# CFD-Xing/gpu-benchmarking

Measured on AMD Instinct MI355X. Metric: GDOF/s for 3D hex sum-factorisation, fp64, nq=2..10 sweep, higher is better.
Workload: dtype f64

## Files before the change

gpu-benchmarking_amd/csrc/bwdtrans_hex.hip:

```cpp
#include "sf_dispatch.h"
#include "wave_launch.h"
#include "wave_table.h"

#include <cstdlib>

namespace sf
{

template <int NQ> struct HexSmall
{
    static constexpr int EC  = HexCfg<NQ>::EC == 1 ? 1
                               : ((HexCfg<NQ>::EC / 4 + 1) / 2 * 2 < 2 ? 2 : (HexCfg<NQ>::EC / 4 + 1) / 2 * 2);
    static constexpr int OUT = HexCfg<NQ>::OUT;
};

__global__ __launch_bounds__(256) void hex_nq2_stream_kernel(const double *__restrict__ b0,
                                                             const double *__restrict__ b1,
                                                             const double *__restrict__ b2,
                                                             const double *__restrict__ in,
                                                             double *__restrict__ out, uint64_t nelmt)
{
    constexpr int U   = 1;
    const uint64_t nv = nelmt * 4;
    const double c0 = b0[0], c1 = b0[1];
    double2_t *out2 = reinterpret_cast<double2_t *>(out);
    const uint64_t base = logical_block<64>() * (256ull * U) + threadIdx.x;
#pragma unroll
    for (int u = 0; u < U; ++u)
    {
        const uint64_t v = base + (uint64_t)u * 256;
        if (v < nv)
        {
            const int p    = (int)(v & 3);
            const double x = in[v >> 2];
            const double bj = b1[p & 1], bk = b2[p >> 1];
            const double2_t r = {((x * c0) * bj) * bk, ((x * c1) * bj) * bk};
            __builtin_nontemporal_store(r, out2 + v);
        }
    }
}

static int launch_hex_nq2(const HexArgs &a, hipStream_t s)
{
    if (a.nelmt == 0)
        return SF_OK;
    const uint64_t blocks = (a.nelmt * 4 + 255) / 256;
    if (blocks > 0x7fffffffull)
        return SF_EINVAL;
    hex_nq2_stream_kernel<<<(unsigned)blocks, 256, 0, s>>>(a.b0, a.b1, a.b2, a.in, a.out, a.nelmt);
    hipError_t e = hipGetLastError();
    return e == hipSuccess ? SF_OK : (int)e;
}

template <int NQ> static int go(const HexArgs &a, hipStream_t s)
{
    if constexpr (NQ == 2)
        return launch_hex_nq2(a, s);
    using C = HexCfg<NQ>;
    constexpr uint64_t per_block = (uint64_t)C::EC * C::WPB * (C::KM > 0 ? C::KM : 1);
    if (a.nelmt < 2 * per_block * (uint64_t)device_info().num_cu)
        return launch_hex_wave<NQ, HexSmall<NQ>::EC, 1, C::BM, C::MW, 1, HexSmall<NQ>::OUT>(a, s);
    constexpr uint64_t piece = hex_piece(NQ);
    if (piece > 0 && a.nelmt > 2 * piece)
    {
        static_assert(piece == 0 || piece % (8 * 64 * per_block) == 0, "pieces hold whole XCD windows");
        constexpr uint64_t NMT = (uint64_t)(NQ - 1) * (NQ - 1) * (NQ - 1), NQT = (uint64_t)NQ * NQ * NQ;
        for (uint64_t lo = 0; lo < a.nelmt; lo += piece)
        {
            HexArgs part = a;
            part.in      = a.in + lo * NMT;
            part.out     = a.out + lo * NQT;
            part.nelmt   = a.nelmt - lo < piece ? a.nelmt - lo : piece;
            const int rc = launch_hex_wave<NQ, C::EC, C::WPB, C::BM, C::MW, C::KM, C::OUT, C::MF>(part, s);
            if (rc != SF_OK)
                return rc;
        }
        return SF_OK;
    }
    return launch_hex_wave<NQ, C::EC, C::WPB, C::BM, C::MW, C::KM, C::OUT, C::MF>(a, s);
}

int launch_hex_wave_nq(unsigned nq, const HexArgs &a, hipStream_t s)
{
    switch (nq)
    {
    case 2: return go<2>(a, s);
    case 3: return go<3>(a, s);
    case 4: return go<4>(a, s);
    case 5: return go<5>(a, s);
    case 6: return go<6>(a, s);
    case 7: return go<7>(a, s);
    case 8: return go<8>(a, s);
    case 9: return go<9>(a, s);
    case 10: return go<10>(a, s);
    case 11: return go<11>(a, s);
    default: return SF_ENOTBUILT;
    }
}

template <int NQ> static int go_mfma(const HexArgs &a, hipStream_t s)
{
    if constexpr (NQ <= 10)
        return launch_hex_mfma<NQ, 2, 2, 2, 1>(a, s);
    else
    {
        constexpr int WPB = NQ == 11 ? 4 : 1;
        constexpr int MW  = (NQ == 14 || NQ == 15) ? 2 : 1;
        return launch_hex_mfma<NQ, 1, WPB, MW, 1, 64>(a, s);
    }
}

int launch_hex_mfma_nq(unsigned nq, const HexArgs &a, hipStream_t s)
{
    switch (nq)
    {
    case 4: return go_mfma<4>(a, s);
    case 5: return go_mfma<5>(a, s);
    case 6: return go_mfma<6>(a, s);
    case 7: return go_mfma<7>(a, s);
    case 8: return go_mfma<8>(a, s);
    case 9: return go_mfma<9>(a, s);
    case 10: return go_mfma<10>(a, s);
    case 11: return go_mfma<11>(a, s);
    case 12: return go_mfma<12>(a, s);
    case 13: return go_mfma<13>(a, s);
    case 14: return go_mfma<14>(a, s);
    case 15: return go_mfma<15>(a, s);
    case 16: return go_mfma<16>(a, s);
    default: return SF_ENOTBUILT;
    }
}

template <int NQ> static int go_mfma4(const HexArgs &a, hipStream_t s)
{
    const char *env = getenv("SF_HEX_MFMA4_CFG");
    const int cfg   = env ? atoi(env) : (NQ == 16 ? 3 : 1);
    if (cfg == 3)
        return launch_hex_mfma4<NQ, 1, 2, 1, 64, true>(a, s);
    return launch_hex_mfma4<NQ, 1, (NQ == 12 ? 1 : 2), 1, 64>(a, s);
}

int launch_hex_mfma4_nq(unsigned nq, const HexArgs &a, hipStream_t s)
{
    switch (nq)
    {
    case 12: return go_mfma4<12>(a, s);
    case 13: return go_mfma4<13>(a, s);
    case 14: return go_mfma4<14>(a, s);
    case 15: return go_mfma4<15>(a, s);
    case 16: return go_mfma4<16>(a, s);
    default: return SF_ENOTBUILT;
    }
}

int hex_auto_kernel(unsigned nq)
{
    return (nq == 12 || nq == 14 || nq == 16) ? SF_VARIANT_MFMA4 : SF_VARIANT_MFMA;
}

typedef float float4_t __attribute__((ext_vector_type(4)));
__global__ __launch_bounds__(256) void hex_nq2_stream_f32_kernel(const float *__restrict__ b0, const float *__restrict__ b1,
                                                                 const float *__restrict__ b2, const float *__restrict__ in,
                                                                 float *__restrict__ out, uint64_t nelmt)
{
    const uint64_t nv = nelmt * 2;
    const uint64_t v  = logical_block<64>() * 256ull + threadIdx.x;
    if (v < nv)
    {
        const float x  = in[v >> 1];
        const float bk = b2[v & 1];
        const float x0 = x * b0[0], x1 = x * b0[1];
        const float4_t r = {(x0 * b1[0]) * bk, (x1 * b1[0]) * bk, (x0 * b1[1]) * bk, (x1 * b1[1]) * bk};
        __builtin_nontemporal_store(r, reinterpret_cast<float4_t *>(out) + v);
    }
}

template <int NQ> static int go_f32(const HexArgsT<float> &a, hipStream_t s)
{
    if constexpr (NQ == 2)
    {
        if (a.nelmt == 0)
            return SF_OK;
        const uint64_t blocks = (a.nelmt * 2 + 255) / 256;
        if (blocks > 0x7fffffffull)
            return SF_EINVAL;
        hex_nq2_stream_f32_kernel<<<(unsigned)blocks, 256, 0, s>>>(a.b0, a.b1, a.b2, a.in, a.out, a.nelmt);
        hipError_t e = hipGetLastError();
        return e == hipSuccess ? SF_OK : (int)e;
    }
    if constexpr (NQ >= 12)
    {
        constexpr int best = NQ == 12 ? 0 : (NQ <= 14 ? 2 : 1);
        static const int cfg = getenv("SF_F32_HEX_CFG") ? atoi(getenv("SF_F32_HEX_CFG")) : best;
        switch (cfg)
        {
        case 1: return launch_hex_mfma<NQ, 1, 1, 1, 1, 64, float>(a, s);
        case 2: return launch_hex_mfma<NQ, 1, 1, 2, 1, 64, float>(a, s);
        case 3: return launch_hex_mfma<NQ, 1, 2, 2, 1, 64, float>(a, s);
        case 4: return launch_hex_mfma<NQ, 2, 1, 1, 1, 64, float>(a, s);
        default: break;
        }
    }
    using C = HexCfgF32<NQ>;
    return launch_hex_wave<NQ, C::EC, C::WPB, C::BM, C::MW, C::KM, C::OUT, C::MF, float>(a, s);
}

int launch_hex_wave_f32_nq(unsigned nq, const HexArgsT<float> &a, hipStream_t s)
{
    switch (nq)
    {
    case 2: return go_f32<2>(a, s);
    case 3: return go_f32<3>(a, s);
    case 4: return go_f32<4>(a, s);
    case 5: return go_f32<5>(a, s);
    case 6: return go_f32<6>(a, s);
    case 7: return go_f32<7>(a, s);
    case 8: return go_f32<8>(a, s);
    case 9: return go_f32<9>(a, s);
    case 10: return go_f32<10>(a, s);
    case 11: return go_f32<11>(a, s);
    case 12: return go_f32<12>(a, s);
    case 13: return go_f32<13>(a, s);
    case 14: return go_f32<14>(a, s);
    case 15: return go_f32<15>(a, s);
    case 16: return go_f32<16>(a, s);
    default: return SF_ENOTBUILT;
    }
}

}
```

gpu-benchmarking_amd/csrc/bwdtrans_wave.h:

```cpp
#pragma once

#include "sf_common.h"

namespace sf
{

enum OutMode
{
    OUT_ST8  = 0,
    OUT_ST16 = 1,
    OUT_LDS  = 2
};

enum BasisMode
{
    BASIS_LDS = 0,
    BASIS_SMEM = 1,
    BASIS_SMEM_COLS = 2,
    BASIS_SMEM_COLS16 = 3
};

template <typename T> struct VecOf
{
    static constexpr int W = 16 / (int)sizeof(T);
    typedef T type __attribute__((ext_vector_type(W)));
};

__device__ __forceinline__ double fma_t(double a, double b, double c)
{
    return __builtin_fma(a, b, c);
}
__device__ __forceinline__ float fma_t(float a, float b, float c)
{
    return __builtin_fmaf(a, b, c);
}

__device__ __forceinline__ double swap_adjacent(double v)
{
    int lo = __double2loint(v), hi = __double2hiint(v);
    lo     = __builtin_amdgcn_mov_dpp(lo, 0xB1, 0xF, 0xF, true);
    hi     = __builtin_amdgcn_mov_dpp(hi, 0xB1, 0xF, 0xF, true);
    return __hiloint2double(hi, lo);
}

template <int NQ, int EC, int DIM, typename T = double> struct WaveGeom
{
    using Scalar = T;
    using Vec    = typename VecOf<T>::type;
    static constexpr int VW  = VecOf<T>::W;
    static constexpr int NM  = NQ - 1;
    static constexpr int NMP = NM | 1;
    static constexpr int NMT = (DIM == 3) ? NM * NM * NM : NM * NM;
    static constexpr int NQT = (DIM == 3) ? NQ * NQ * NQ : NQ * NQ;
    static constexpr int IN_STRIDE = (NM % 2 == 0) ? NM + 1 : NM;
    static constexpr int IN_DBL    = EC * NMT;
    static constexpr bool VEC2     = (IN_DBL % VW) == 0;
    static constexpr int P0 = (DIM == 3) ? EC * NM * NM : EC * NM;
    static constexpr int P1 = (DIM == 3) ? EC * NQ * NM : EC * NQ;
    static constexpr int P2 = EC * NQ * NQ;
    static constexpr int PASS0 = cdiv(P0, kWave);
    static constexpr int PASS1 = cdiv(P1, kWave);
    static constexpr int PASS2 = cdiv(P2, kWave);
    static constexpr int SLAB_IN = P0 * IN_STRIDE;
    static constexpr int SLAB_W1 = P1 * NMP;
    static constexpr int SLAB_W2 = (DIM == 3) ? P2 * NMP : 0;
    static constexpr int SLAB0   = CMax<CMax<SLAB_IN, SLAB_W1>::value, SLAB_W2>::value;
    static constexpr int OUT_DBL = EC * NQT;
    static constexpr int SLAB_NOOUT = (SLAB0 + VW - 1) / VW * VW;
    static constexpr int SLAB_OUT   = (CMax<SLAB0, OUT_DBL>::value + VW - 1) / VW * VW;
    static constexpr int NBAS = (NM * NQ + VW - 1) / VW * VW;
    static constexpr int NLD  = VEC2 ? cdiv(IN_DBL / VW, kWave) : cdiv(IN_DBL, kWave);
    static constexpr bool ALIGN_OK = VEC2 && cdiv(IN_DBL / VW + 7, kWave) == NLD;
};

__device__ __forceinline__ int align_shift(const void *p)
{
    return __builtin_amdgcn_readfirstlane((int)(((uintptr_t)p >> 4) & 7));
}

template <class G, int OUTM> constexpr int slab_doubles()
{
    return OUTM == OUT_LDS ? G::SLAB_OUT : G::SLAB_NOOUT;
}

template <int NQ, int EC, int DIM, int WPB, int BMODE, int OUTM, typename T = double>
constexpr size_t wave_lds_bytes()
{
    using G = WaveGeom<NQ, EC, DIM, T>;
    return sizeof(T) *
           (size_t)((BMODE == BASIS_LDS ? DIM * G::NBAS : 0) + WPB * slab_doubles<G, OUTM>());
}

struct ChunkIter
{
    uint64_t first, step, count;
};

template <int KMAP, int WPB, int XG = 0>
__device__ __forceinline__ ChunkIter chunk_iter(uint64_t nchunk, int wib)
{
    const uint64_t gw = logical_block<XG>() * WPB + wib;
    ChunkIter it;
    if constexpr (KMAP == 0)
    {
        const uint64_t nwave = (uint64_t)gridDim.x * WPB;
        it.first = gw;
        it.step  = nwave;
        it.count = gw < nchunk ? (nchunk - gw + nwave - 1) / nwave : 0;
    }
    else if constexpr (KMAP > 0)
    {
        it.first = gw * KMAP;
        it.step  = 1;
        it.count = it.first < nchunk ? (nchunk - it.first < KMAP ? nchunk - it.first : KMAP) : 0;
    }
    else
    {
        constexpr int K     = -KMAP;
        const uint64_t base = logical_block<XG>() * WPB * K;
        it.first            = base + wib;
        it.step             = WPB;
        const uint64_t end  = base + (uint64_t)WPB * K < nchunk ? base + (uint64_t)WPB * K : nchunk;
        it.count            = it.first < end ? (end - it.first + WPB - 1) / WPB : 0;
    }
    return it;
}

template <typename T> __device__ __forceinline__ int line_offset(const void *p)
{
    return __builtin_amdgcn_readfirstlane((int)(((uintptr_t)p / sizeof(T)) & (128 / sizeof(T) - 1)));
}
__device__ __forceinline__ int line_offset_f64(const void *p)
{
    return line_offset<double>(p);
}

template <int NMAX, typename T> constexpr int word_grid_regs()
{
    return cdiv(NMAX + (int)(128 / sizeof(T)) - 1, (int)(16 / sizeof(T)) * kWave);
}

template <int NMAX, int NREG, typename T>
__device__ __forceinline__ void chunk_load_any(typename VecOf<T>::type (&st)[NREG], const T *__restrict__ src,
                                               int lane, int nvalid)
{
    using V          = typename VecOf<T>::type;
    constexpr int VW = VecOf<T>::W;
    constexpr int NLDA = word_grid_regs<NMAX, T>();
    static_assert(NLDA <= NREG, "staging registers");
    const int a   = line_offset<T>(src);
    const V *grid = reinterpret_cast<const V *>(src - a);
#pragma unroll
    for (int k = 0; k < NLDA; ++k)
    {
        const int gv = k * kWave + lane;
        const int d0 = VW * gv - a;
        V x          = {};
        if (d0 >= 0 && d0 + VW - 1 < nvalid)
            x = __builtin_nontemporal_load(grid + gv);
        else
        {
#pragma unroll
            for (int h = 0; h < VW; ++h)
                if (d0 + h >= 0 && d0 + h < nvalid)
                    x[h] = src[d0 + h];
        }
        st[k] = x;
    }
}

template <int NMAX, int NREG>
__device__ __forceinline__ void chunk_load_any_f64(double2_t (&st)[NREG], const double *__restrict__ src,
                                                   int lane, int nvalid)
{
    chunk_load_any<NMAX, NREG, double>(st, src, lane, nvalid);
}

template <typename V, int N> __device__ __forceinline__ void touch_staged(V (&st)[N])
{
#pragma unroll
    for (int k = 0; k < N; ++k)
        asm volatile("" : "+v"(st[k]));
}

template <class G, bool FULL, bool NTL = true, bool AL = false>
__device__ __forceinline__ void chunk_load(typename G::Vec (&st)[G::NLD],
                                           const typename G::Scalar *__restrict__ src, int lane,
                                           int nvalid )
{
    using T = typename G::Scalar;
    using V = typename G::Vec;
    constexpr int VW = G::VW;
    if constexpr (G::VEC2)
    {
        const V *srcv = reinterpret_cast<const V *>(src);
        const int sh  = AL ? align_shift(src) : 0;
#pragma unroll
        for (int k = 0; k < G::NLD; ++k)
        {
            const int v = k * kWave + lane - sh;
            if constexpr (FULL)
            {
                if (AL ? (v >= 0 && v < G::IN_DBL / VW)
                       : ((k + 1) * kWave <= G::IN_DBL / VW || v < G::IN_DBL / VW))
                    st[k] = NTL ? __builtin_nontemporal_load(srcv + v) : srcv[v];
            }
            else
            {
                V x = {};
                if (AL && v < 0)
                    ;
                else if (VW * v + VW - 1 < nvalid)
                    x = NTL ? __builtin_nontemporal_load(srcv + v) : srcv[v];
                else
                {
#pragma unroll
                    for (int j = 0; j < VW - 1; ++j)
                        if (VW * v + j < nvalid)
                            x[j] = src[VW * v + j];
                }
                st[k] = x;
            }
        }
    }
    else
    {
        chunk_load_any<G::IN_DBL, G::NLD, T>(st, src, lane, FULL ? G::IN_DBL : nvalid);
    }
}

template <class G, bool AL = false>
__device__ __forceinline__ void chunk_stage(const typename G::Vec (&st)[G::NLD],
                                            typename G::Scalar *slab, int lane, int sh = 0)
{
    using V = typename G::Vec;
    constexpr int VW = G::VW;
    if constexpr (G::VEC2)
    {
#pragma unroll
        for (int k = 0; k < G::NLD; ++k)
        {
            const int v = k * kWave + lane - (AL ? sh : 0);
            if (AL ? (v >= 0 && v < G::IN_DBL / VW)
                   : ((k + 1) * kWave <= G::IN_DBL / VW || v < G::IN_DBL / VW))
            {
                if constexpr (G::IN_STRIDE == G::NM)
                {
                    *reinterpret_cast<V *>(slab + VW * v) = st[k];
                }
                else
                {
#pragma unroll
                    for (int j = 0; j < VW; ++j)
                    {
                        const int f          = VW * v + j;
                        slab[f + f / G::NM] = st[k][j];
                    }
                }
            }
        }
    }
    else
    {
#pragma unroll
        for (int k = 0; k < word_grid_regs<G::IN_DBL, typename G::Scalar>(); ++k)
#pragma unroll
            for (int h = 0; h < VW; ++h)
            {
                const int f = VW * (k * kWave + lane) - sh + h;
                if (f >= 0 && f < G::IN_DBL)
                {
                    if constexpr (G::IN_STRIDE == G::NM)
                        slab[f] = st[k][h];
                    else
                        slab[f + f / G::NM] = st[k][h];
                }
            }
    }
}

typedef float float2_t __attribute__((ext_vector_type(2)));
template <int NB, int N0, int NOUT, int NPASS>
__device__ __forceinline__ void fma_row(bool first, const double (&um)[NPASS], const double (&b)[NB],
                                        double (&acc)[NPASS][NOUT])
{
#pragma unroll
    for (int n = 0; n < NB; ++n)
#pragma unroll
        for (int s = 0; s < NPASS; ++s)
            acc[s][N0 + n] = first ? um[s] * b[n] : fma_t(um[s], b[n], acc[s][N0 + n]);
}
template <int NB, int N0, int NOUT, int NPASS>
__device__ __forceinline__ void fma_row(bool first, const float (&um)[NPASS], const float (&b)[NB],
                                        float (&acc)[NPASS][NOUT])
{
    constexpr int NPAIR = (NOUT >= 9 && NOUT <= 24) ? NB / 2 : 0;
#pragma unroll
    for (int n = 0; n < 2 * NPAIR; n += 2)
#pragma unroll
        for (int s = 0; s < NPASS; ++s)
        {
            const float2_t uu = {um[s], um[s]}, bb = {b[n], b[n + 1]};
            const float2_t a  = {acc[s][N0 + n], acc[s][N0 + n + 1]};
            const float2_t r  = first ? uu * bb : __builtin_elementwise_fma(uu, bb, a);
            acc[s][N0 + n]     = r.x;
            acc[s][N0 + n + 1] = r.y;
        }
#pragma unroll
    for (int n = 2 * NPAIR; n < NB; ++n)
#pragma unroll
        for (int s = 0; s < NPASS; ++s)
            acc[s][N0 + n] = first ? um[s] * b[n] : fma_t(um[s], b[n], acc[s][N0 + n]);
}

template <int NIN, int NOUT, int NPASS, int N0, int kColBlock, typename T>
__device__ __forceinline__ void contract_cols(const T (&u)[NPASS][NIN], T (&acc)[NPASS][NOUT],
                                              const T *__restrict__ bas, int &zero)
{
    constexpr int NB = (NOUT - N0) < kColBlock ? (NOUT - N0) : kColBlock;
    T b[2][NB];
#pragma unroll
    for (int n = 0; n < NB; ++n)
        b[0][n] = bas[zero + N0 + n];
#pragma unroll
    for (int m = 0; m < NIN; ++m)
    {
#pragma unroll
        for (int n = 0; n < NB; ++n)
            asm volatile("" : "+s"(zero) : "s"(b[m % 2][n]));
        if (m + 1 < NIN)
        {
#pragma unroll
            for (int n = 0; n < NB; ++n)
                b[(m + 1) % 2][n] = bas[zero + (m + 1) * NOUT + N0 + n];
            __builtin_amdgcn_sched_barrier(0);
        }
        {
            T um[NPASS];
#pragma unroll
            for (int s = 0; s < NPASS; ++s)
                um[s] = u[s][m];
            fma_row<NB, N0>(m == 0, um, b[m % 2], acc);
        }
#pragma unroll
        for (int n = 0; n < NB; ++n)
#pragma unroll
            for (int s = 0; s < NPASS; ++s)
                asm volatile("" : "+s"(zero) : "v"(acc[s][N0 + n]));
    }
    if constexpr (N0 + NB < NOUT)
        contract_cols<NIN, NOUT, NPASS, N0 + NB, kColBlock, T>(u, acc, bas, zero);
}

template <int NIN, int NOUT, int NPASS, int BMODE, typename T>
__device__ __forceinline__ void contract(const T (&u)[NPASS][NIN], T (&acc)[NPASS][NOUT],
                                         const T *__restrict__ bas)
{
    if constexpr (BMODE == BASIS_SMEM_COLS || BMODE == BASIS_SMEM_COLS16)
    {
        int z = 0;
        asm volatile("s_mov_b32 %0, 0" : "=s"(z));
        contract_cols<NIN, NOUT, NPASS, 0, (BMODE == BASIS_SMEM_COLS ? 8 : 16), T>(u, acc, bas, z);
        return;
    }
    int zero = 0;
    asm volatile("s_mov_b32 %0, 0" : "=s"(zero));
    constexpr int RING = 2;
    T b[RING][NOUT];
#pragma unroll
    for (int n = 0; n < NOUT; ++n)
        b[0][n] = bas[zero + n];
#pragma unroll
    for (int m = 0; m < NIN; ++m)
    {
        if constexpr (BMODE == BASIS_SMEM)
        {
#pragma unroll
            for (int n = 0; n < NOUT; ++n)
                asm volatile("" : "+s"(zero) : "s"(b[m % RING][n]));
        }
        if (m + 1 < NIN)
        {
#pragma unroll
            for (int n = 0; n < NOUT; ++n)
                b[(m + 1) % RING][n] = bas[zero + (m + 1) * NOUT + n];
            __builtin_amdgcn_sched_barrier(0);
        }
        {
            T um[NPASS];
#pragma unroll
            for (int s = 0; s < NPASS; ++s)
                um[s] = u[s][m];
            fma_row<NOUT, 0>(m == 0, um, b[m % RING], acc);
        }
#pragma unroll
        for (int n = 0; n < NOUT; ++n)
#pragma unroll
            for (int s = 0; s < NPASS; ++s)
                asm volatile("" : "+s"(zero) : "v"(acc[s][n]));
    }
}

template <int NIN, int NPASS, int NP, int STRIDE, typename T>
__device__ __forceinline__ void read_pencils(T (&u)[NPASS][NIN], const T *slab, int lane)
{
#pragma unroll
    for (int s = 0; s < NPASS; ++s)
    {
        int t = s * kWave + lane;
        if ((s + 1) * kWave > NP)
            t = t < NP ? t : NP - 1;
#pragma unroll
        for (int m = 0; m < NIN; ++m)
            u[s][m] = slab[t * STRIDE + m];
    }
}

template <class G, int DIM, int WPB, int BMODE, int SLAB, typename T>
__device__ __forceinline__ T *wave_setup(T *lds, const T *const (&gb)[3], const T *(&bs)[3], int wib)
{
    if constexpr (BMODE == BASIS_LDS)
    {
        for (int x = threadIdx.x; x < G::NM * (G::NM + 1); x += kWave * WPB)
#pragma unroll
            for (int d = 0; d < DIM; ++d)
                lds[d * G::NBAS + x] = gb[d][x];
        __syncthreads();
#pragma unroll
        for (int d = 0; d < DIM; ++d)
            bs[d] = lds + d * G::NBAS;
        return lds + DIM * G::NBAS + wib * SLAB;
    }
    else
    {
#pragma unroll
        for (int d = 0; d < DIM; ++d)
            bs[d] = gb[d];
        return lds + wib * SLAB;
    }
}

template <class G, int EC, bool NTL = true, bool AL = false>
__device__ __forceinline__ void chunk_fetch(typename G::Vec (&st)[G::NLD],
                                            const typename G::Scalar *__restrict__ in, uint64_t c,
                                            uint64_t nelmt, int lane)
{
    const uint64_t left = nelmt - c * EC;
    if (left >= EC)
        chunk_load<G, true, NTL, AL>(st, in + c * G::IN_DBL, lane, 0);
    else
        chunk_load<G, false, NTL, AL>(st, in + c * G::IN_DBL, lane, (int)left * G::NMT);
}

template <int NOUT, int NSTRIDE, bool ST16, bool NTS = true, typename T>
__device__ __forceinline__ void store_column(const T (&acc)[NOUT], T *dst, int lane)
{
    if constexpr (ST16)
    {
        static_assert(sizeof(T) == 8, "paired 16-byte stores are the fp64 path");
        static_assert(NOUT % 2 == 0 && NSTRIDE % 2 == 0, "16-byte stores need even extents");
        const bool odd = lane & 1;
        double *d2     = dst - (odd ? 1 : 0) + (odd ? NSTRIDE : 0);
#pragma unroll
        for (int n = 0; n < NOUT; n += 2)
        {
            const double give = odd ? acc[n] : acc[n + 1];
            const double got  = swap_adjacent(give);
            double2_t v;
            v.x = odd ? got : acc[n];
            v.y = odd ? acc[n + 1] : got;
            if (NTS)
                __builtin_nontemporal_store(v, reinterpret_cast<double2_t *>(d2 + n * NSTRIDE));
            else
                *reinterpret_cast<double2_t *>(d2 + n * NSTRIDE) = v;
        }
    }
    else
    {
#pragma unroll
        for (int n = 0; n < NOUT; ++n)
        {
            if (NTS)
                __builtin_nontemporal_store(acc[n], dst + n * NSTRIDE);
            else
                dst[n * NSTRIDE] = acc[n];
        }
    }
}

template <int NMAX, typename T>
__device__ __forceinline__ void flush_any(const T *img, T *__restrict__ dst, int nout, int lane)
{
    using V          = typename VecOf<T>::type;
    constexpr int VW = VecOf<T>::W;
    const int a      = line_offset<T>(dst);
    V *grid          = reinterpret_cast<V *>(dst - a);
    constexpr int NST = word_grid_regs<NMAX, T>();
#pragma unroll
    for (int k = 0; k < NST; ++k)
    {
        const int gv = k * kWave + lane;
        const int d0 = VW * gv - a;
        if (d0 >= 0 && d0 + VW - 1 < nout)
        {
            V x;
#pragma unroll
            for (int h = 0; h < VW; ++h)
                x[h] = img[d0 + h];
            __builtin_nontemporal_store(x, grid + gv);
        }
        else
        {
#pragma unroll
            for (int h = 0; h < VW; ++h)
                if (d0 + h >= 0 && d0 + h < nout)
                    dst[d0 + h] = img[d0 + h];
        }
    }
}

template <int NMAX>
__device__ __forceinline__ void flush_any_f64(const double *img, double *__restrict__ dst, int nout, int lane)
{
    flush_any<NMAX, double>(img, dst, nout, lane);
}

template <class G, bool NTS, bool AL = false>
__device__ __forceinline__ void chunk_flush(const typename G::Scalar *slab,
                                            typename G::Scalar *__restrict__ dst, int nout, int lane)
{
    using V = typename G::Vec;
    constexpr int VW = G::VW;
    if constexpr (G::OUT_DBL % VW == 0)
    {
        constexpr int NST = cdiv(G::OUT_DBL / VW + (AL ? 7 : 0), kWave);
        V *dstv           = reinterpret_cast<V *>(dst);
        const int sh      = AL ? align_shift(dst) : 0;
#pragma unroll
        for (int k = 0; k < NST; ++k)
        {
            const int v = k * kWave + lane - sh;
            if (AL && v < 0)
                continue;
            if (VW * v + VW - 1 < nout)
            {
                const V x = *reinterpret_cast<const V *>(slab + VW * v);
                if (NTS)
                    __builtin_nontemporal_store(x, dstv + v);
                else
                    dstv[v] = x;
            }
            else
            {
#pragma unroll
                for (int j = 0; j < VW - 1; ++j)
                    if (VW * v + j < nout)
                        dst[VW * v + j] = slab[VW * v + j];
            }
        }
    }
    else
    {
        flush_any<G::OUT_DBL, typename G::Scalar>(slab, dst, nout, lane);
    }
}

template <class G, int WPB, int SLAB>
__device__ __forceinline__ void block_load_stage(typename G::Scalar *slab0, const typename G::Scalar *__restrict__ src,
                                                 int nvalid)
{
    using T          = typename G::Scalar;
    using V          = typename G::Vec;
    constexpr int VW = G::VW;
    constexpr int NB = WPB * G::IN_DBL;
    constexpr int NT = WPB * kWave;
    constexpr int NW = cdiv(cdiv(NB + (int)(128 / sizeof(T)) - 1, VW), NT);
    const int a      = line_offset<T>(src);
    const V *grid    = reinterpret_cast<const V *>(src - a);
    V x[NW];
#pragma unroll
    for (int k = 0; k < NW; ++k)
    {
        const int gv = k * NT + (int)threadIdx.x;
        const int d0 = VW * gv - a;
        V v          = {};
        if (d0 >= 0 && d0 + VW - 1 < nvalid)
            v = __builtin_nontemporal_load(grid + gv);
        else
        {
#pragma unroll
            for (int h = 0; h < VW; ++h)
                if (d0 + h >= 0 && d0 + h < nvalid)
                    v[h] = src[d0 + h];
        }
        x[k] = v;
    }
#pragma unroll
    for (int k = 0; k < NW; ++k)
#pragma unroll
        for (int h = 0; h < VW; ++h)
        {
            const int f = VW * (k * NT + (int)threadIdx.x) - a + h;
            if (f >= 0 && f < NB)
            {
                const int w = f / G::IN_DBL, r = f - w * G::IN_DBL;
                T *dst      = slab0 + w * SLAB;
                if constexpr (G::IN_STRIDE == G::NM)
                    dst[r] = x[k][h];
                else
                    dst[r + r / G::NM] = x[k][h];
            }
        }
}

template <int NQ, int EC, int WPB, int BMODE, int MINW, int KMAP, int OUTM, int MEMF = 0,
          typename T = double>
__global__ __launch_bounds__(kWave *WPB, MINW) void hex_wave_kernel(
    const T *__restrict__ b0, const T *__restrict__ b1, const T *__restrict__ b2,
    const T *__restrict__ in, T *__restrict__ out, uint64_t nelmt)
{
    using G          = WaveGeom<NQ, EC, 3, T>;
    constexpr int NM = G::NM, NMP = G::NMP, NM2 = NM * NM, NQ2 = NQ * NQ;
    static_assert(OUTM != OUT_ST16 || (NQ % 2 == 0 && sizeof(T) == 8),
                  "paired 16-byte stores need even nq and fp64");
    constexpr int SLAB = slab_doubles<G, OUTM>();

    extern __shared__ __attribute__((aligned(16))) unsigned char lds_raw[];
    T *lds = reinterpret_cast<T *>(lds_raw);
    const int lane = threadIdx.x & (kWave - 1);
    const int wib  = __builtin_amdgcn_readfirstlane(threadIdx.x >> 6);
    const T *const gb[3] = {b0, b1, b2};
    const T *bs[3];
    T *slab = wave_setup<G, 3, WPB, BMODE, SLAB>(lds, gb, bs, wib);

    constexpr int XG  = (MEMF >> 4) & 0xfff;
    constexpr bool BL = ((MEMF >> 16) & 1) != 0;
    static_assert(!BL || (KMAP == 1 && BMODE != BASIS_LDS), "cooperative input: one chunk per wave, basis in SGPRs");
    const uint64_t nchunk = (nelmt + EC - 1) / EC;
    const ChunkIter it    = chunk_iter<KMAP, WPB, XG>(nchunk, wib);
    if constexpr (BL)
    {
        const uint64_t first = logical_block<XG>() * (uint64_t)(WPB * EC);
        if (first < nelmt)
        {
            const uint64_t left = nelmt - first;
            block_load_stage<G, WPB, SLAB>(lds, in + first * G::NMT,
                                           left >= (uint64_t)(WPB * EC) ? WPB * G::IN_DBL : (int)left * G::NMT);
        }
        __syncthreads();
    }
    if (it.count == 0)
        return;

    constexpr bool AL = (MEMF & 4) && G::ALIGN_OK;
    typename G::Vec st[BL ? 1 : G::NLD];
    if constexpr (!BL)
        chunk_fetch<G, EC, !(MEMF & 1), AL>(st, in, it.first, nelmt, lane);

    uint64_t c = it.first;
    for (uint64_t n = 0; n < it.count; ++n, c += it.step)
    {
        const uint64_t left = nelmt - c * EC;
        const int evalid    = left >= EC ? EC : (int)left;

        if constexpr (!BL)
        {
            chunk_stage<G, AL>(st, slab, lane,
                               G::VEC2 ? (AL ? align_shift(in + c * G::IN_DBL) : 0)
                                       : line_offset<T>(in + c * G::IN_DBL));
            wave_lds_fence();

            if (n + 1 < it.count)
                chunk_fetch<G, EC, !(MEMF & 1), AL>(st, in, c + it.step, nelmt, lane);
        }

        {
            T u[G::PASS0][NM], acc[G::PASS0][NQ];
            read_pencils<NM, G::PASS0, G::P0, G::IN_STRIDE>(u, slab, lane);
            contract<NM, NQ, G::PASS0, BMODE>(u, acc, bs[0]);
            wave_lds_fence();
#pragma unroll
            for (int s = 0; s < G::PASS0; ++s)
            {
                const int t = s * kWave + lane;
                if ((s + 1) * kWave <= G::P0 || t < G::P0)
                {
                    const int e = t / NM2, rq = t - e * NM2, r = rq / NM, q = rq - r * NM;
                    T *dst = slab + (e * NQ * NM + r) * NMP + q;
#pragma unroll
                    for (int i = 0; i < NQ; ++i)
                        dst[i * NM * NMP] = acc[s][i];
                }
            }
            wave_lds_fence();
        }
        {
            T u[G::PASS1][NM], acc[G::PASS1][NQ];
            read_pencils<NM, G::PASS1, G::P1, NMP>(u, slab, lane);
            contract<NM, NQ, G::PASS1, BMODE>(u, acc, bs[1]);
            wave_lds_fence();
#pragma unroll
            for (int s = 0; s < G::PASS1; ++s)
            {
                const int t = s * kWave + lane;
                if ((s + 1) * kWave <= G::P1 || t < G::P1)
                {
                    const int e = t / (NQ * NM), ir = t - e * (NQ * NM), i = ir / NM,
                              r = ir - i * NM;
                    T *dst = slab + (e * NQ2 + i) * NMP + r;
#pragma unroll
                    for (int j = 0; j < NQ; ++j)
                        dst[j * NQ * NMP] = acc[s][j];
                }
            }
            wave_lds_fence();
        }
        {
            T u[G::PASS2][NM], acc[G::PASS2][NQ];
            read_pencils<NM, G::PASS2, G::P2, NMP>(u, slab, lane);
            contract<NM, NQ, G::PASS2, BMODE>(u, acc, bs[2]);
            T *oc = out + c * (uint64_t)(EC * G::NQT);
            if constexpr (OUTM == OUT_LDS)
            {
                wave_lds_fence();
#pragma unroll
                for (int s = 0; s < G::PASS2; ++s)
                {
                    const int t = s * kWave + lane;
                    if ((s + 1) * kWave <= G::P2 || t < G::P2)
                    {
                        const int e = t / NQ2, pl = t - e * NQ2;
                        T *dst = slab + e * G::NQT + pl;
#pragma unroll
                        for (int k = 0; k < NQ; ++k)
                            dst[k * NQ2] = acc[s][k];
                    }
                }
                wave_lds_fence();
                chunk_flush<G, !(MEMF & 2), (MEMF & 8) != 0>(slab, oc, evalid * G::NQT, lane);
            }
            else
            {
#pragma unroll
                for (int s = 0; s < G::PASS2; ++s)
                {
                    const int t = s * kWave + lane;
                    const int e = t / NQ2, pl = t - e * NQ2;
                    if (((s + 1) * kWave <= G::P2 || t < G::P2) && e < evalid)
                        store_column<NQ, NQ2, OUTM == OUT_ST16, !(MEMF & 2)>(
                            acc[s], oc + e * G::NQT + pl, lane);
                }
            }
            wave_lds_fence();
        }
    }
}

template <int NQ, int EC, int WPB, int BMODE, int MINW, int KMAP, int OUTM, int MEMF = 0,
          typename T = double>
__global__ __launch_bounds__(kWave *WPB, MINW) void quad_wave_kernel(
    const T *__restrict__ b0, const T *__restrict__ b1, const T *__restrict__ in,
    T *__restrict__ out, uint64_t nelmt)
{
    using G          = WaveGeom<NQ, EC, 2, T>;
    constexpr int NM = G::NM, NMP = G::NMP;
    static_assert(OUTM != OUT_ST16 || (NQ % 2 == 0 && sizeof(T) == 8),
                  "paired 16-byte stores need even nq and fp64");
    constexpr int SLAB = slab_doubles<G, OUTM>();

    extern __shared__ __attribute__((aligned(16))) unsigned char lds_raw[];
    T *lds = reinterpret_cast<T *>(lds_raw);
    const int lane = threadIdx.x & (kWave - 1);
    const int wib  = __builtin_amdgcn_readfirstlane(threadIdx.x >> 6);
    const T *const gb[3] = {b0, b1, nullptr};
    const T *bs[3];
    T *slab = wave_setup<G, 2, WPB, BMODE, SLAB>(lds, gb, bs, wib);

    const uint64_t nchunk = (nelmt + EC - 1) / EC;
    const ChunkIter it    = chunk_iter<KMAP, WPB, ((MEMF >> 4) & 0xfff)>(nchunk, wib);
    if (it.count == 0)
        return;

    constexpr bool AL = (MEMF & 4) && G::ALIGN_OK;
    typename G::Vec st[G::NLD];
    chunk_fetch<G, EC, !(MEMF & 1), AL>(st, in, it.first, nelmt, lane);

    uint64_t c = it.first;
    for (uint64_t n = 0; n < it.count; ++n, c += it.step)
    {
        const uint64_t left = nelmt - c * EC;
        const int evalid    = left >= EC ? EC : (int)left;

        chunk_stage<G, AL>(st, slab, lane,
                           G::VEC2 ? (AL ? align_shift(in + c * G::IN_DBL) : 0)
                                   : line_offset<T>(in + c * G::IN_DBL));
        wave_lds_fence();
        if (n + 1 < it.count)
            chunk_fetch<G, EC, !(MEMF & 1), AL>(st, in, c + it.step, nelmt, lane);

        {
            T u[G::PASS0][NM], acc[G::PASS0][NQ];
            read_pencils<NM, G::PASS0, G::P0, G::IN_STRIDE>(u, slab, lane);
            contract<NM, NQ, G::PASS0, BMODE>(u, acc, bs[0]);
            wave_lds_fence();
#pragma unroll
            for (int s = 0; s < G::PASS0; ++s)
            {
                const int t = s * kWave + lane;
                if ((s + 1) * kWave <= G::P0 || t < G::P0)
                {
                    const int e = t / NM, q = t - e * NM;
                    T *dst = slab + e * NQ * NMP + q;
#pragma unroll
                    for (int i = 0; i < NQ; ++i)
                        dst[i * NMP] = acc[s][i];
                }
            }
            wave_lds_fence();
        }
        {
            T u[G::PASS1][NM], acc[G::PASS1][NQ];
            read_pencils<NM, G::PASS1, G::P1, NMP>(u, slab, lane);
            contract<NM, NQ, G::PASS1, BMODE>(u, acc, bs[1]);
            T *oc = out + c * (uint64_t)(EC * G::NQT);
            if constexpr (OUTM == OUT_LDS)
            {
                wave_lds_fence();
#pragma unroll
                for (int s = 0; s < G::PASS1; ++s)
                {
                    const int t = s * kWave + lane;
                    if ((s + 1) * kWave <= G::P1 || t < G::P1)
                    {
                        const int e = t / NQ, i = t - e * NQ;
                        T *dst = slab + e * G::NQT + i;
#pragma unroll
                        for (int j = 0; j < NQ; ++j)
                            dst[j * NQ] = acc[s][j];
                    }
                }
                wave_lds_fence();
                chunk_flush<G, !(MEMF & 2), (MEMF & 8) != 0>(slab, oc, evalid * G::NQT, lane);
            }
            else
            {
#pragma unroll
                for (int s = 0; s < G::PASS1; ++s)
                {
                    const int t = s * kWave + lane;
                    const int e = t / NQ, i = t - e * NQ;
                    if (((s + 1) * kWave <= G::P1 || t < G::P1) && e < evalid)
                        store_column<NQ, NQ, OUTM == OUT_ST16, !(MEMF & 2)>(
                            acc[s], oc + e * G::NQT + i, lane);
                }
            }
            wave_lds_fence();
        }
    }
}

}
```

gpu-benchmarking_amd/csrc/wave_table.h:

```cpp
#pragma once
#include "bwdtrans_wave.h"

namespace sf
{

constexpr int XG16 = 16 << 4, XG64 = 64 << 4;

template <int NQ> struct HexCfg;
#define SF_HEX_CFG(NQ_, EC_, WPB_, BM_, MW_, KM_, OUT_, MF_)                                        \
    template <> struct HexCfg<NQ_>                                                                 \
    {                                                                                              \
        static constexpr int EC = EC_, WPB = WPB_, BM = BM_, MW = MW_, KM = KM_;                   \
        static constexpr int OUT = OUT_, MF = MF_;                                                      \
    }
SF_HEX_CFG(2,  128, 4, BASIS_SMEM, 2, 1, OUT_ST16, 0);
SF_HEX_CFG(3,  14,  2, BASIS_SMEM, 2, 1, OUT_LDS, XG64 | 8);
SF_HEX_CFG(4,  4,   8, BASIS_SMEM, 4, 1, OUT_LDS, XG64);
SF_HEX_CFG(5,  2,   4, BASIS_SMEM, 2, 1, OUT_LDS, XG64 | 8);
SF_HEX_CFG(6,  2,   8, BASIS_SMEM, 2, 1, OUT_LDS, XG64);
SF_HEX_CFG(7,  1,   4, BASIS_SMEM, 4, 1, OUT_LDS, XG64 | 8);
SF_HEX_CFG(8,  1,   8, BASIS_SMEM, 4, 1, OUT_LDS, XG64);
SF_HEX_CFG(9,  1,   4, BASIS_SMEM, 4, 1, OUT_LDS, XG64 | 8);
SF_HEX_CFG(10, 1,   4, BASIS_SMEM, 4, 1, OUT_LDS, XG64 | 8);
SF_HEX_CFG(11, 1,   4, BASIS_SMEM, 1, 1, OUT_LDS, XG64);
#undef SF_HEX_CFG

constexpr uint64_t hex_piece(int nq)
{
    return (nq == 7 || nq == 8) ? (1ull << 19) : 0;
}

template <int NQ> struct QuadCfg;
#define SF_QUAD_CFG(NQ_, EC_, WPB_, BM_, MW_, KM_, OUT_, MF_)                                       \
    template <> struct QuadCfg<NQ_>                                                                \
    {                                                                                              \
        static constexpr int EC = EC_, WPB = WPB_, BM = BM_, MW = MW_, KM = KM_, OUT = OUT_;       \
        static constexpr int MF = MF_;                                                             \
    }
SF_QUAD_CFG(2,  128, 4, BASIS_SMEM, 2, 1, OUT_LDS, 0);
SF_QUAD_CFG(3,  42,  4, BASIS_SMEM, 2, 1, OUT_LDS, 8);
SF_QUAD_CFG(4,  16,  4, BASIS_SMEM, 2, 1, OUT_LDS, XG64);
SF_QUAD_CFG(5,  8,   4, BASIS_SMEM, 4, 1, OUT_LDS, XG64 | 8);
SF_QUAD_CFG(6,  8,   4, BASIS_SMEM, 4, 1, OUT_LDS, XG64);
SF_QUAD_CFG(7,  6,   4, BASIS_SMEM, 4, 1, OUT_LDS, XG64 | 12);
SF_QUAD_CFG(8,  4,   4, BASIS_SMEM, 4, 1, OUT_LDS, XG64);
SF_QUAD_CFG(9,  4,   4, BASIS_SMEM, 2, 1, OUT_LDS, 8);
SF_QUAD_CFG(10, 4,   8, BASIS_SMEM, 2, 1, OUT_LDS, XG64);
SF_QUAD_CFG(11, 4,   4, BASIS_SMEM_COLS, 2, 1, OUT_LDS, XG64 | 8);
SF_QUAD_CFG(12, 3,   4, BASIS_SMEM_COLS16, 2, 1, OUT_LDS, XG64);
SF_QUAD_CFG(13, 4,   4, BASIS_SMEM_COLS16, 2, 1, OUT_LDS, XG64 | 12);
SF_QUAD_CFG(14, 4,   4, BASIS_SMEM_COLS16, 2, 1, OUT_LDS, XG64);
SF_QUAD_CFG(15, 4,   8, BASIS_SMEM_COLS16, 2, 1, OUT_LDS, XG64 | 12);
SF_QUAD_CFG(16, 4,   4, BASIS_SMEM_COLS16, 2, 1, OUT_LDS, XG64);
SF_QUAD_CFG(17, 3,   4, BASIS_SMEM_COLS16, 2, 1, OUT_LDS,  XG64);
SF_QUAD_CFG(18, 3,   4, BASIS_SMEM_COLS16, 2, 1, OUT_LDS,  XG64);
SF_QUAD_CFG(19, 3,   4, BASIS_SMEM_COLS16, 2, 1, OUT_LDS,  XG64);
SF_QUAD_CFG(20, 3,   4, BASIS_SMEM_COLS16, 2, 1, OUT_LDS,  XG64);
SF_QUAD_CFG(21, 3,   4, BASIS_SMEM_COLS16, 2, 1, OUT_ST8,  XG64);
SF_QUAD_CFG(22, 2,   4, BASIS_SMEM_COLS16, 2, 1, OUT_LDS,  XG64);
SF_QUAD_CFG(23, 2,   4, BASIS_SMEM_COLS16, 2, 1, OUT_ST8,  XG64);
SF_QUAD_CFG(24, 2,   4, BASIS_SMEM_COLS16, 2, 1, OUT_ST16, XG64);
SF_QUAD_CFG(32, 2,   4, BASIS_SMEM_COLS16, 1, 2, OUT_ST16, 0);
#undef SF_QUAD_CFG

constexpr int hex_f32_mf(int nq)
{
    return ((nq % 2 && nq >= 3) ? 8 : 0) | (nq >= 7 ? XG64 : 0);
}
constexpr int quad_f32_mf(int nq)
{
    return (nq == 15 ? 12 : ((nq == 7 || nq == 9 || nq == 11) ? 8 : 0)) | (nq >= 12 ? XG64 : 0);
}
template <int NQ> struct HexCfgF32
{
    static constexpr int EC = 2 * HexCfg<NQ>::EC, WPB = HexCfg<NQ>::WPB, BM = HexCfg<NQ>::BM;
    static constexpr int MW = HexCfg<NQ>::MW >= 2 ? 4 : 2, KM = 1, OUT = OUT_LDS, MF = hex_f32_mf(NQ);
};
template <> struct HexCfgF32<3>
{
    static constexpr int EC = 28, WPB = 4, BM = BASIS_SMEM, MW = 4, KM = 1, OUT = OUT_LDS, MF = 8;
};
template <> struct HexCfgF32<6>
{
    static constexpr int EC = 4, WPB = 4, BM = BASIS_SMEM, MW = 4, KM = 1, OUT = OUT_LDS, MF = 0;
};
template <> struct HexCfgF32<7>
{
    static constexpr int EC = 4, WPB = 4, BM = BASIS_SMEM, MW = 4, KM = 1, OUT = OUT_LDS, MF = XG64 | 8;
};
template <> struct HexCfgF32<9>
{
    static constexpr int EC = 4, WPB = 2, BM = BASIS_SMEM, MW = 2, KM = 1, OUT = OUT_LDS, MF = XG64 | 8;
};
template <int NQ> struct QuadCfgF32
{
    static constexpr int EC = 2 * QuadCfg<NQ>::EC, WPB = QuadCfg<NQ>::WPB, BM = QuadCfg<NQ>::BM;
    static constexpr int MW = QuadCfg<NQ>::MW >= 2 ? 4 : 2, KM = 1, OUT = OUT_LDS, MF = quad_f32_mf(NQ);
};

#define SF_QUAD_F32_LOW(NQ_, EC_, MW_)                                                             \
    template <> struct QuadCfgF32<NQ_>                                                             \
    {                                                                                              \
        static constexpr int EC = EC_, WPB = 4, BM = BASIS_SMEM, MW = MW_, KM = 1, OUT = OUT_LDS, MF = XG64; \
    }
SF_QUAD_F32_LOW(4, 32, 4);
SF_QUAD_F32_LOW(6, 16, 4);
SF_QUAD_F32_LOW(8, 8, 4);
SF_QUAD_F32_LOW(10, 8, 4);
#undef SF_QUAD_F32_LOW

#define SF_QUAD_F32_ODD(NQ_, EC_, BM_, MW_, MF_)                                                   \
    template <> struct QuadCfgF32<NQ_>                                                             \
    {                                                                                              \
        static constexpr int EC = EC_, WPB = 4, BM = BM_, MW = MW_, KM = 1, OUT = OUT_LDS, MF = MF_; \
    }
SF_QUAD_F32_ODD(5, 16, BASIS_SMEM, 4, XG64 | 8);
SF_QUAD_F32_ODD(7, 16, BASIS_SMEM, 4, XG64 | 8);
SF_QUAD_F32_ODD(9, 8, BASIS_SMEM, 4, 8);
SF_QUAD_F32_ODD(11, 8, BASIS_SMEM_COLS, 4, XG64 | 8);
#undef SF_QUAD_F32_ODD

#define SF_QUAD_F32(NQ_, EC_, MW_, MF_)                                                            \
    template <> struct QuadCfgF32<NQ_>                                                             \
    {                                                                                              \
        static constexpr int EC = EC_, WPB = 4, BM = BASIS_SMEM_COLS16, MW = MW_, KM = 1, OUT = OUT_LDS, MF = MF_; \
    }
SF_QUAD_F32(12, 4, 4, XG64);
SF_QUAD_F32(13, 16, 2, XG64 | 12);
SF_QUAD_F32(14, 4, 4, XG64);
SF_QUAD_F32(15, 4, 4, XG64 | 12);
SF_QUAD_F32(16, 4, 4, XG64);
SF_QUAD_F32(20, 8, 4, XG64);
SF_QUAD_F32(25, 2, 4, XG64 | 8);
SF_QUAD_F32(26, 2, 4, XG64);
SF_QUAD_F32(27, 2, 4, XG64 | 8);
SF_QUAD_F32(28, 2, 4, XG64);
SF_QUAD_F32(29, 2, 4, XG64 | 8);
SF_QUAD_F32(30, 2, 4, XG64);
SF_QUAD_F32(31, 2, 4, XG64 | 8);
#undef SF_QUAD_F32

#define SF_HEX_F32(NQ_, WPB_, MW_, MF_)                                                            \
    template <> struct HexCfgF32<NQ_>                                                              \
    {                                                                                              \
        static constexpr int EC = 1, WPB = WPB_, BM = BASIS_SMEM, MW = MW_, KM = 1, OUT = OUT_LDS, MF = MF_; \
    }
SF_HEX_F32(12, 4, 2, XG64);
SF_HEX_F32(13, 4, 2, XG64 | 8);
SF_HEX_F32(14, 4, 2, XG64);
SF_HEX_F32(15, 2, 2, XG64 | 8);
SF_HEX_F32(16, 2, 2, XG64);
#undef SF_HEX_F32

}
```

Baseline: 317.9.

## Prime basis rows into a scalar register ring and retune small hex dispatch

Adds a primed scalar-register ring that prefetches basis rows for the next contraction pass while the current one computes, used for nq=7 and nq=8 in the small-element path. It also widens the small-case threshold for nq=8 and adds a mid-size path for nq=8 with four waves per block and priming enabled. The aim is to hide scalar basis-load latency behind the FMAs and to pick better launch shapes at moderate element counts. Optional timestamp instrumentation is compiled in only under SF_WAVE_STAMP. The cost is extra scalar register pressure and more template variants.

```diff
diff --git a/gpu-benchmarking_amd/csrc/bwdtrans_hex.hip b/gpu-benchmarking_amd/csrc/bwdtrans_hex.hip
--- a/gpu-benchmarking_amd/csrc/bwdtrans_hex.hip
+++ b/gpu-benchmarking_amd/csrc/bwdtrans_hex.hip
@@ -12,6 +12,7 @@
     static constexpr int EC  = HexCfg<NQ>::EC == 1 ? 1
                                : ((HexCfg<NQ>::EC / 4 + 1) / 2 * 2 < 2 ? 2 : (HexCfg<NQ>::EC / 4 + 1) / 2 * 2);
     static constexpr int OUT = HexCfg<NQ>::OUT;
+    static constexpr int MF = hex_small_mf(NQ);
 };
 
 __global__ __launch_bounds__(256) void hex_nq2_stream_kernel(const double *__restrict__ b0,
@@ -58,8 +59,16 @@
         return launch_hex_nq2(a, s);
     using C = HexCfg<NQ>;
     constexpr uint64_t per_block = (uint64_t)C::EC * C::WPB * (C::KM > 0 ? C::KM : 1);
-    if (a.nelmt < 2 * per_block * (uint64_t)device_info().num_cu)
-        return launch_hex_wave<NQ, HexSmall<NQ>::EC, 1, C::BM, C::MW, 1, HexSmall<NQ>::OUT>(a, s);
+    const uint64_t num_cu = (uint64_t)device_info().num_cu;
+    const uint64_t small_below = hex_small_waves(NQ) ? (uint64_t)hex_small_waves(NQ) * 4 * HexSmall<NQ>::EC * num_cu + 1
+                                                     : 2 * per_block * num_cu;
+    if (a.nelmt < small_below)
+        return launch_hex_wave<NQ, HexSmall<NQ>::EC, 1, C::BM, C::MW, 1, HexSmall<NQ>::OUT, HexSmall<NQ>::MF>(a, s);
+    if constexpr (hex_mid_wpb(NQ) > 0)
+    {
+        if (a.nelmt < hex_mid_below(NQ))
+            return launch_hex_wave<NQ, C::EC, hex_mid_wpb(NQ), C::BM, C::MW, C::KM, C::OUT, C::MF | BPRIME>(a, s);
+    }
     constexpr uint64_t piece = hex_piece(NQ);
     if (piece > 0 && a.nelmt > 2 * piece)
     {
diff --git a/gpu-benchmarking_amd/csrc/bwdtrans_wave.h b/gpu-benchmarking_amd/csrc/bwdtrans_wave.h
--- a/gpu-benchmarking_amd/csrc/bwdtrans_wave.h
+++ b/gpu-benchmarking_amd/csrc/bwdtrans_wave.h
@@ -401,6 +401,59 @@
     }
 }
 
+template <int NOUT, int RING, typename T>
+__device__ __forceinline__ void ring_request(T (&b)[RING][NOUT], const T *__restrict__ bas, int &zero, int s, int m0,
+                                             int cnt)
+{
+#pragma unroll
+    for (int m = m0; m < m0 + cnt; ++m)
+#pragma unroll
+        for (int n = 0; n < NOUT; ++n)
+            b[(s + m) % RING][n] = bas[zero + m * NOUT + n];
+    __builtin_amdgcn_sched_barrier(0);
+}
+
+template <int NIN, int NOUT, int NPASS, int RING, int S, bool NEXT, typename T>
+__device__ __forceinline__ void contract_ring(const T (&u)[NPASS][NIN], T (&acc)[NPASS][NOUT],
+                                              const T *__restrict__ bas, const T *__restrict__ nxt,
+                                              T (&b)[RING][NOUT], int &zero)
+{
+    constexpr int GROUP = RING / 2, NG = cdiv(NIN, GROUP);
+    static_assert(RING % 2 == 0 && NIN >= RING, "ring = two groups of rows");
+#pragma unroll
+    for (int g = 0; g < NG; ++g)
+    {
+        const int m0 = g * GROUP, cnt = NIN - m0 < GROUP ? NIN - m0 : GROUP;
+#pragma unroll
+        for (int m = m0; m < m0 + cnt; ++m)
+#pragma unroll
+            for (int n = 0; n < NOUT; ++n)
+                asm volatile("" : "+s"(zero) : "s"(b[(S + m) % RING][n]));
+        if (g == 0 && NG > 1)
+            ;
+        else if (g + 1 < NG)
+            ring_request<NOUT, RING>(b, bas, zero, S, m0 + GROUP, NIN - m0 - GROUP < GROUP ? NIN - m0 - GROUP : GROUP);
+        else if (NEXT)
+            ring_request<NOUT, RING>(b, nxt, zero, (S + NIN) % RING, 0, GROUP);
+#pragma unroll
+        for (int m = m0; m < m0 + cnt; ++m)
+        {
+            T um[NPASS];
+#pragma unroll
+            for (int s = 0; s < NPASS; ++s)
+                um[s] = u[s][m];
+            fma_row<NOUT, 0>(m == 0, um, b[(S + m) % RING], acc);
+#pragma unroll
+            for (int n = 0; n < NOUT; ++n)
+#pragma unroll
+                for (int s = 0; s < NPASS; ++s)
+                    asm volatile("" : "+s"(zero) : "v"(acc[s][n]));
+        }
+    }
+    if (NEXT)
+        ring_request<NOUT, RING>(b, nxt, zero, (S + NIN) % RING, GROUP, GROUP);
+}
+
 template <int NIN, int NPASS, int NP, int STRIDE, typename T>
 __device__ __forceinline__ void read_pencils(T (&u)[NPASS][NIN], const T *slab, int lane)
 {
@@ -613,6 +666,19 @@
         }
 }
 
+template <typename T, int A, int B> __device__ __forceinline__ void touch_all(T (&x)[A][B])
+{
+#pragma unroll
+    for (int a = 0; a < A; ++a)
+#pragma unroll
+        for (int b = 0; b < B; ++b)
+            asm volatile("" : "+v"(x[a][b]));
+}
+
+#ifdef SF_WAVE_STAMP
+__device__ unsigned long long *sf_wave_stamps;
+#endif
+
 template <int NQ, int EC, int WPB, int BMODE, int MINW, int KMAP, int OUTM, int MEMF = 0,
           typename T = double>
 __global__ __launch_bounds__(kWave *WPB, MINW) void hex_wave_kernel(
@@ -624,6 +690,26 @@
     static_assert(OUTM != OUT_ST16 || (NQ % 2 == 0 && sizeof(T) == 8),
                   "paired 16-byte stores need even nq and fp64");
     constexpr int SLAB = slab_doubles<G, OUTM>();
+    constexpr bool PRIME = ((MEMF >> 17) & 1) != 0 && BMODE == BASIS_SMEM;
+    constexpr int GROUP = 1 + ((MEMF >> 18) & 3), RING = 2 * GROUP;
+    constexpr bool WARM = ((MEMF >> 21) & 1) != 0;
+    static_assert(PRIME || (((MEMF >> 17) & 7) == 0 && !WARM), "the primed ring needs scalar-operand rows");
+#ifdef SF_WAVE_STAMP
+    constexpr bool STAMP = ((MEMF >> 20) & 1) != 0;
+    static_assert(!STAMP || KMAP == 1, "stamps: one chunk per wave");
+#else
+    constexpr bool STAMP = false;
+#endif
+    unsigned long long tstamp[STAMP ? 11 : 1];
+    auto stamp = [&](int k) {
+        if constexpr (STAMP)
+        {
+            __builtin_amdgcn_sched_barrier(0);
+            tstamp[k] = __builtin_amdgcn_s_memtime();
+            __builtin_amdgcn_sched_barrier(0);
+        }
+    };
+    stamp(0);
 
     extern __shared__ __attribute__((aligned(16))) unsigned char lds_raw[];
     T *lds = reinterpret_cast<T *>(lds_raw);
@@ -657,11 +743,49 @@
     if constexpr (!BL)
         chunk_fetch<G, EC, !(MEMF & 1), AL>(st, in, it.first, nelmt, lane);
 
+    T ring[PRIME ? RING : 1][NQ];
+    int zero = 0;
+    if constexpr (PRIME)
+    {
+        asm volatile("s_mov_b32 %0, 0" : "=s"(zero));
+        constexpr int NLINE = WARM ? cdiv(NM * NQ * (int)sizeof(T), 64) : 0;
+        int warm[3][NLINE + 1];
+        if constexpr (WARM)
+        {
+#pragma unroll
+            for (int d = 0; d < 3; ++d)
+#pragma unroll
+                for (int l = 0; l <= NLINE; ++l)
+                    warm[d][l] = reinterpret_cast<const int *>(bs[d])[zero + (l < NLINE ? l * 16 : NM * NQ * (int)sizeof(T) / 4 - 1)];
+        }
+        ring_request<NQ, RING>(ring, bs[0], zero, 0, 0, RING);
+        if constexpr (WARM)
+        {
+#pragma unroll
+            for (int d = 0; d < 3; ++d)
+#pragma unroll
+                for (int l = 0; l <= NLINE; ++l)
+                    asm volatile("" : "+s"(zero) : "s"(warm[d][l]));
+        }
+#pragma unroll
+        for (int m = 0; m < RING; ++m)
+#pragma unroll
+            for (int n = 0; n < NQ; ++n)
+                asm volatile("" : "+s"(zero) : "s"(ring[m][n]));
+    }
+
     uint64_t c = it.first;
     for (uint64_t n = 0; n < it.count; ++n, c += it.step)
     {
         const uint64_t left = nelmt - c * EC;
         const int evalid    = left >= EC ? EC : (int)left;
+
+        stamp(1);
+        if constexpr (STAMP && !BL)
+        {
+            touch_staged(st);
+            stamp(2);
+        }
 
         if constexpr (!BL)
         {
@@ -677,7 +801,20 @@
         {
             T u[G::PASS0][NM], acc[G::PASS0][NQ];
             read_pencils<NM, G::PASS0, G::P0, G::IN_STRIDE>(u, slab, lane);
-            contract<NM, NQ, G::PASS0, BMODE>(u, acc, bs[0]);
+            if constexpr (STAMP)
+            {
+                touch_all(u);
+                stamp(3);
+            }
+            if constexpr (PRIME)
+                contract_ring<NM, NQ, G::PASS0, RING, 0, true>(u, acc, bs[0], bs[1], ring, zero);
+            else
+                contract<NM, NQ, G::PASS0, BMODE>(u, acc, bs[0]);
+            if constexpr (STAMP)
+            {
+                touch_all(acc);
+                stamp(4);
+            }
             wave_lds_fence();
 #pragma unroll
             for (int s = 0; s < G::PASS0; ++s)
@@ -697,7 +834,20 @@
         {
             T u[G::PASS1][NM], acc[G::PASS1][NQ];
             read_pencils<NM, G::PASS1, G::P1, NMP>(u, slab, lane);
-            contract<NM, NQ, G::PASS1, BMODE>(u, acc, bs[1]);
+            if constexpr (STAMP)
+            {
+                touch_all(u);
+                stamp(5);
+            }
+            if constexpr (PRIME)
+                contract_ring<NM, NQ, G::PASS1, RING, NM % RING, true>(u, acc, bs[1], bs[2], ring, zero);
+            else
+                contract<NM, NQ, G::PASS1, BMODE>(u, acc, bs[1]);
+            if constexpr (STAMP)
+            {
+                touch_all(acc);
+                stamp(6);
+            }
             wave_lds_fence();
 #pragma unroll
             for (int s = 0; s < G::PASS1; ++s)
@@ -718,7 +868,20 @@
         {
             T u[G::PASS2][NM], acc[G::PASS2][NQ];
             read_pencils<NM, G::PASS2, G::P2, NMP>(u, slab, lane);
-            contract<NM, NQ, G::PASS2, BMODE>(u, acc, bs[2]);
+            if constexpr (STAMP)
+            {
+                touch_all(u);
+                stamp(7);
+            }
+            if constexpr (PRIME)
+                contract_ring<NM, NQ, G::PASS2, RING, (2 * NM) % RING, false>(u, acc, bs[2], bs[2], ring, zero);
+            else
+                contract<NM, NQ, G::PASS2, BMODE>(u, acc, bs[2]);
+            if constexpr (STAMP)
+            {
+                touch_all(acc);
+                stamp(8);
+            }
             T *oc = out + c * (uint64_t)(EC * G::NQT);
             if constexpr (OUTM == OUT_LDS)
             {
@@ -753,7 +916,27 @@
             }
             wave_lds_fence();
         }
-    }
+        if constexpr (PRIME && KMAP != 1)
+        {
+            asm volatile("s_mov_b32 %0, 0" : "=s"(zero));
+            ring_request<NQ, RING>(ring, bs[0], zero, 0, 0, RING);
+        }
+    }
+#ifdef SF_WAVE_STAMP
+    if constexpr (STAMP)
+    {
+        stamp(9);
+        __builtin_amdgcn_s_waitcnt(0x0f70);
+        stamp(10);
+        if (lane == 0 && sf_wave_stamps)
+        {
+            unsigned long long *mine = sf_wave_stamps + ((uint64_t)blockIdx.x * WPB + wib) * 16;
+#pragma unroll
+            for (int k = 0; k < 11; ++k)
+                mine[k] = tstamp[k];
+        }
+    }
+#endif
 }
 
 template <int NQ, int EC, int WPB, int BMODE, int MINW, int KMAP, int OUTM, int MEMF = 0,
diff --git a/gpu-benchmarking_amd/csrc/wave_table.h b/gpu-benchmarking_amd/csrc/wave_table.h
--- a/gpu-benchmarking_amd/csrc/wave_table.h
+++ b/gpu-benchmarking_amd/csrc/wave_table.h
@@ -5,6 +5,7 @@
 {
 
 constexpr int XG16 = 16 << 4, XG64 = 64 << 4;
+constexpr int BPRIME = 1 << 17, BROWS2 = 1 << 18, BWARM = 1 << 21;
 
 template <int NQ> struct HexCfg;
 #define SF_HEX_CFG(NQ_, EC_, WPB_, BM_, MW_, KM_, OUT_, MF_)                                        \
@@ -28,6 +29,23 @@
 constexpr uint64_t hex_piece(int nq)
 {
     return (nq == 7 || nq == 8) ? (1ull << 19) : 0;
+}
+
+constexpr int hex_small_mf(int nq)
+{
+    return nq == 8 ? (BPRIME | BROWS2) : (nq == 7 ? BPRIME : 0);
+}
+constexpr int hex_small_waves(int nq)
+{
+    return nq == 8 ? 6 : 0;
+}
+constexpr int hex_mid_wpb(int nq)
+{
+    return nq == 8 ? 4 : 0;
+}
+constexpr uint64_t hex_mid_below(int nq)
+{
+    return nq == 8 ? 196608 : 0;
 }
 
 template <int NQ> struct QuadCfg;
```

After: 317.5. About the same (-0.1%).
